# olsonanl/signature_kmers

Hardware: AMD Instinct MI355X
Metric: k-mers/sec (extract+hash+count) at 1/2/4/8 GPUs; achieved HBM GB/s % (higher is better)
Workload: dtype u8

## Files before the change

signature_kmers_amd/__init__.py:

```python
from __future__ import annotations

import ctypes as C
import os
from dataclasses import dataclass

import numpy as np

__all__ = [
    "SkmError", "lib", "K", "UNDEFINED_FUNCTION", "STORED_DTYPE", "CALL_DTYPE",
    "SignatureBuilder", "KeptKmers", "CmphKmerDb", "FunctionCaller", "mph_build",
    "kmer_to_str", "str_to_kmer", "keys_from_strings", "device_count", "MatrixDistance", "SeqIdMap",
    "matrix_tile_rows",
]

K = 8
UNDEFINED_FUNCTION = 0xFFFF
_HERE = os.path.dirname(os.path.abspath(__file__))
LIB_PATH = os.environ.get("SKM_LIB_PATH") or os.path.join(_HERE, "libskm.so")

STORED_DTYPE = np.dtype([("avg_from_end", "<u2"), ("function_index", "<u2"), ("mean", "<u2"),
                         ("median", "<u2"), ("var", "<u2")])
CALL_DTYPE = np.dtype([("start", "<u4"), ("end", "<u4"), ("count", "<i4"), ("function_index", "<u2"),
                       ("pad", "<u2"), ("protein_length_median", "<u4"),
                       ("protein_length_med_avg_dev", "<f4")])
# ... 280 lines not shown
            return {}
        ms = (C.c_float * n)()
        cnt = (C.c_uint64 * n)()
        buf = C.create_string_buffer(64 * n + 64)
        lib().skm_build_kernel_timings(self._h, buf, len(buf), ms, cnt, n)
        names = buf.value.decode().split("\n")[:n]
        return {names[i]: (float(ms[i]), int(cnt[i])) for i in range(n)}

    def set_option(self, name: str, value: int):
        _check(lib().skm_build_set_option(self._h, name.encode(), int(value)))

    def passes(self) -> int:
        return self.counters()["passes"]

    def counters(self) -> dict:
        v = (C.c_uint64 * 48)()
        n = lib().skm_build_counters(self._h, v, 48)
        names = ["windows", "kept", "overflow_subbuckets", "chain_jobs", "chain_samples", "sequences", "grouped",
                 "overflow_elements", "overflow_kept", "big_groups", "big_kept", "passes", "valid", "giant_chains",
                 "giant_max", "redone", "cap_overflow_scratch", "cap_split", "cap_long_samples", "cap_long_jobs",
                 "demand_overflow_scratch", "demand_split", "demand_long_samples", "demand_long_jobs",
                 "long_samples", "routed", "add_batch_us", "prepare_upload_us", "prepare_plan_us", "prepare_rest_us",
                 "pass_groups", "add_pack_us", "add_dma_wait_us", "finish_us", "finish_wait_us", "finish_copy_us",
                 "finish_chunks", "finish_select_dev_us", "finish_sort_dev_us", "finish_gather_dev_us",
                 "finish_d2h_dev_us", "finish_max_chunk", "finish_wide_index", "kept_cap",
                 "free_after_prepare", "recs_rot", "overflow_light_subbuckets", "overflow_light_elements"]
        return {names[i]: int(v[i]) for i in range(n)}

    def debug_jobs(self, k: int = 64) -> list:
        v = (C.c_uint32 * k)()
        _check(lib().skm_build_debug_jobs(self._h, v, k))
        return [int(x) for x in v]

    def debug_overflow(self, k: int = 4096) -> list:
        v = (C.c_uint32 * k)()
        n = lib().skm_build_debug_overflow(self._h, v, k)
        return [int(x) for x in v[:min(max(n, 0), k)]]

    def debug_stamps(self, enable: bool) -> list:
        v = (C.c_uint64 * 32)()
        _check(lib().skm_build_debug_stamps(self._h, 1 if enable else 0, v, 32))
# ... 554 lines not shown
```

signature_kmers_amd/csrc/skm_build.hip:

```cpp
#include <hip/hip_runtime.h>

#include <algorithm>
#include <type_traits>
#include <chrono>
#include <cmath>
#include <cstdio>
#include <cstdlib>
#include <cstring>
#include <deque>
#include <functional>
#include <memory>
#include <numeric>
#include <string>
#include <thread>
#include <vector>

#include "skm_common.h"
#include "skm_pool.h"
#include "skm_output.h"
#include "skm_util.h"

#if defined(SKM_WITH_RCCL)
#include <rccl/rccl.h>
#endif
// ... 342 lines not shown
            }
}

__device__ __forceinline__ void stats_small(GRes& r, uint32_t x0, uint32_t x1, uint32_t n) {
    r.median = 0;
    r.var = 0;
    if (n == 2) {
        const uint16_t sum = (uint16_t)(x0 + x1);
        const double mean = (double)sum / 2.0;
        const double tmp = (double)x1 - mean;
        const double v = 0.0 * 1.0 / 2.0 + tmp * tmp / 1.0;
        r.var = d2u16(v);
    }
}

__device__ __forceinline__ void mark_seq(uint8_t* f, uint32_t s) {
    const uintptr_t p = reinterpret_cast<uintptr_t>(f);
    if (p & 1u) {
        uint32_t* w = reinterpret_cast<uint32_t*>(p & ~(uintptr_t)1) + (s >> 5);
        const uint32_t m = 1u << (s & 31u);
        if (!(*w & m)) atomicOr(w, m);
    } else {
        f[s] = 1;
    }
}

template <int N>
__device__ __forceinline__ void mark_seqs(uint8_t* f, int flag_check, const uint32_t (&s)[N]) {
    const uintptr_t p = reinterpret_cast<uintptr_t>(f);
    if (p & 1u) {
        uint32_t* w = reinterpret_cast<uint32_t*>(p & ~(uintptr_t)1);
        uint32_t cur[N];
#pragma unroll
        for (int u = 0; u < N; ++u) cur[u] = s[u] != 0xFFFFFFFFu ? w[s[u] >> 5] : 0xFFFFFFFFu;
#pragma unroll
        for (int u = 0; u < N; ++u) {
            const uint32_t m = 1u << (s[u] & 31u);
            if (!(cur[u] & m)) atomicOr(w + (s[u] >> 5), m);
        }
    } else {
        uint8_t cur[N];
#pragma unroll
        for (int u = 0; u < N; ++u) cur[u] = s[u] != 0xFFFFFFFFu && flag_check ? f[s[u]] : (uint8_t)(s[u] == 0xFFFFFFFFu);
#pragma unroll
        for (int u = 0; u < N; ++u)
            if (cur[u] == 0) f[s[u]] = 1;
    }
}

template <int N, class V>
__device__ GRes group_thread(const V& v, uint64_t a, uint32_t c, const uint32_t* __restrict__ glen,
                             uint8_t* __restrict__ flags) {
    GRes r;
    r.kept = false;
    uint32_t fn[N], of[N];
#pragma unroll
    for (int t = 0; t < N; ++t) {
        if ((uint32_t)t < c) {
            fn[t] = v.func(a + t);
            of[t] = (uint32_t)(v.lov(a + t) & 0xFFFFu);
        } else {
            fn[t] = 0x10000u;
            of[t] = 0x10000u;
        }
    }
    uint32_t best_f = fn[0], best_c = 0, rb = 0, run_s = 0;
#pragma unroll
// ... 34 lines not shown
            sum += len;
            const uint32_t q = rb + best_c - 1 - t;
            if (q == 0) lr0 = len;
            if (q == 1) lr1 = len;
        }
    }
    r.mean = d2u16((double)(uint16_t)sum / (double)best_c);
    r.median = 0;
    r.var = 0;
    if (best_c <= 2) stats_small(r, lr0, lr1, best_c);
    return r;
}

template <class V>
__device__ GRes group_wave(const V& v, uint64_t a, uint32_t c, const uint32_t* __restrict__ glen,
                           uint8_t* __restrict__ flags) {
    const uint32_t lane = threadIdx.x & 63u;
    GRes r;
    r.kept = false;
    uint32_t best_f = 0, best_c = 0, rb = 0, run_s = 0;
    uint32_t run_f = v.func(a);
    for (uint32_t base = 0; base < c; base += 64) {
        const uint32_t t = base + lane;
        const bool valid = t < c;
        const uint32_t f = valid ? v.func(a + t) : 0xFFFFFFFFu;
        const uint32_t fp = (valid && t > 0) ? v.func(a + t - 1) : 0xFFFFFFFFu;
        uint64_t m = __ballot(valid && t > 0 && f != fp);
        while (m) {
            const int q = __ffsll((long long)m) - 1;
            m &= m - 1;
            const uint32_t pos = base + (uint32_t)q;
// ... 76 lines not shown
}

__device__ __forceinline__ uint32_t wg_min(uint32_t x, uint32_t* s_wave) {
    const uint32_t lane = threadIdx.x & 63u, wave = threadIdx.x >> 6, nw = blockDim.x >> 6;
    x = wave_min(x);
    if (lane == 0) s_wave[wave] = x;
    __syncthreads();
    uint32_t t = 0xFFFFFFFFu;
    for (uint32_t w = 0; w < nw; ++w) t = min(t, s_wave[w]);
    __syncthreads();
    return t;
}

template <class V>
__device__ bool group_block(const V& v, uint64_t a, uint32_t c, const uint32_t* __restrict__ glen,
                            uint8_t* __restrict__ flags, uint32_t* heads, uint32_t hcap, uint32_t* s_wave, GRes& r) {
    const uint32_t tid = threadIdx.x, nt = blockDim.x;
    r.kept = false;
    uint32_t H = 0;
    for (uint32_t t0 = 0; t0 < c; t0 += nt) {
        const uint32_t t = t0 + tid;
        const bool head = t < c && (t == 0 || v.func(a + t) != v.func(a + t - 1));
        uint32_t tot;
        const uint32_t pos = wg_exclusive_scan(head ? 1u : 0u, s_wave, tot);
        if (head && H + pos < hcap) heads[H + pos] = t;
        H += tot;
    }
    if (H > hcap) return false;
    __syncthreads();
    uint32_t lmax = 0;
    for (uint32_t j = tid; j < H; j += nt) lmax = max(lmax, (j + 1 < H ? heads[j + 1] : c) - heads[j]);
// ... 48 lines not shown
    RUN_LONG_WANT = 12,
    RUN_LONG_WANTJ = 13,
    RUN_ACC_LIGHT_SUB = 14,
    RUN_ACC_LIGHT_ELEMS = 15,
    RUN_ACC_NOVF = 16,
    RUN_ACC_JOBS = 17,
    RUN_ACC_LENS = 18,
    RUN_ACC_OVF_ELEMS = 19,
    RUN_ACC_OVF_KEPT = 20,
    RUN_ACC_BIG = 21,
    RUN_ACC_BIG_KEPT = 22,
    RUN_ACC_GROUPED = 23,
    RUN_LAST_NOVF = 24,
    RUN_LAST_JOBS = 25,
    RUN_NLOC = 26,
    RUN_SLOTS = 64
};
constexpr unsigned long long RUN_F_ARENA = 1;
constexpr unsigned long long RUN_F_RERUN = 2;
constexpr unsigned long long RUN_F_CAP = 4;
enum : uint32_t {
    PLAN_NOVF = 0,
    PLAN_NSPLIT = 1,
    PLAN_NHEAVY = 2,
    PLAN_SKIP = 3,
    PLAN_Q_SPLIT = 4,
    PLAN_Q_HEAVY = 5,
    PLAN_Q_REST = 6,
    PLAN_Q_LIGHT = 7,
    PLAN_SLOTS = 8
// ... 1536 lines not shown
    uint64_t* recs_hi;
    const uint64_t* recs_lo;
    uint64_t* tmp_hi;
    uint64_t* tmp_lo;
    const uint64_t* bstart;
    const uint64_t* seg_start;
    const uint32_t* seg_len;
    uint32_t nsrc;
    uint32_t* sub_tab;
    unsigned long long* kept_ctr;

    uint32_t nbuckets;
    uint32_t bucket_base;
    int rem_bits;
    const uint32_t* glen;
    uint8_t* flags;
    unsigned long long* ctr;
    uint64_t* out_keys;
    skm_stored_kmer_data* out_data;
    Job* jobs;
    uint32_t* lens;
    OvfEntry* ovf;
    uint32_t ovf_cap;
    unsigned long long* stamps;
    uint64_t* big_desc;
    uint32_t big_cap;
    unsigned long long* big_ctr;
    int prio;
    int pshift;
    int flag_check;
    const uint32_t* skip;
// ... 134 lines not shown
        const uint32_t g = L.big[q];
        rep = L.glist[g];
        a = L.goff[rep];
        c = (g + 1 < G ? L.goff[L.glist[g + 1]] : M) - a;
    }
    const bool real = gv && m < c;
    uint64_t key = ~0ull;
    uint32_t pay = 0;
    if (real) {
        const uint32_t j = L.order[a + m];
        const uint64_t hj = L.hi[j], lj = L.lo[j];
        key = ((hj & 0xFFFFull) << 48) | (lj >> 16);
        pay = (uint32_t)(hj >> 47);
    }
    key = seg_bitonic64<S>(key, pay, m);
    const uint32_t f = (uint32_t)(key >> 48);
    const uint32_t fprev = (uint32_t)__shfl_up((int)f, 1, 64);
    const bool head = !real || m == 0 || f != fprev;
    const uint64_t H = __ballot(head);
    const uint64_t above = lane == 63 ? 0ull : (H & ~((2ull << lane) - 1ull));
    const uint32_t nh = above ? (uint32_t)__ffsll((long long)above) - 1u : 64u;
    const uint32_t rlen = min(nh, sbase + c) - lane;
    const uint32_t v = (real && head) ? ((rlen << 16) | (0xFFFFu - f)) : 0u;
    const uint32_t best = seg_reduce_max<S>(v);
    const uint32_t cbest = best >> 16, bf = 0xFFFFu - (best & 0xFFFFu);
    const bool kept = gv && !((float)cbest < float(c) * 0.8f);
    const bool inrun = real && f == bf;
    const uint32_t len16 = pay >> 1;
    const uint32_t sum = seg_reduce_sum<S>(inrun ? len16 : 0u);
    const uint32_t i = (uint32_t)(key & ((1u << ELEM_I_BITS) - 1));
    const uint32_t off = real ? ((len16 - i) & 0xFFFFu) : 0x10000u;
    const uint32_t osort = seg_bitonic32<S>(off, m);
    const uint32_t avg = (uint32_t)__shfl((int)osort, (int)(sbase + (c >> 1)), 64);
    const uint64_t R = __ballot(inrun);
    const uint64_t segmask = (S == 64) ? ~0ull : (((1ull << S) - 1ull) << sbase);
    const uint64_t Rs = R & segmask;
    const uint32_t rs = Rs ? (uint32_t)__ffsll((long long)Rs) - 1u : sbase;
    const uint32_t s = (uint32_t)(key >> ELEM_I_BITS) & ((1u << ELEM_S_BITS) - 1u);
    const uint32_t fl = (A.flag_check && real && A.flags) ? A.flags[s] : 0u;
    const uint32_t len = (pay & 1u) ? A.glen[s] : len16;
    if (kept && real && fl == 0 && A.flags) mark_seq(A.flags, s);
    const uint32_t x0 = (uint32_t)__shfl((int)len, (int)(rs + cbest - 1), 64);
    const uint32_t x1 = (uint32_t)__shfl((int)len, (int)rs, 64);
    if (kept && inrun && cbest >= 3) L.lens32[2 * a + (rs + cbest - 1 - lane)] = len;
    if (kept && m == 0) {
        GRes r;
        r.kept = true;
        r.best_f = bf;
        r.cbest = cbest;
        r.avg = avg;
        r.mean = d2u16((double)(uint16_t)sum / (double)cbest);
        stats_small(r, x0, cbest == 2 ? x1 : 0u, cbest);
        const uint64_t h43 = key_h43(hprefix, (L.hi[rep] >> 16) & REM_MASK, A.rem_bits, A.pshift);
        L.hi[rep] = kept_hi(h43, r.avg);
        if (cbest >= 3) {
            jobinfo[rep] = (a << 16) | JOB_KEPT | cbest;
            fmean[rep] = bf | ((uint32_t)r.mean << 16);
        } else {
            jobinfo[rep] = JOB_KEPT;
// ... 287 lines not shown
    return L;
}

__global__ __launch_bounds__(BPK_THREADS, BPK_WAVES_EU) void k_bucket_process(BucketArgs A) {
    static_assert(CAP % BPK_THREADS == 0, "emit assigns CAP / BPK_THREADS elements per thread");
    __shared__ SubMem s_mem;
    __shared__ uint32_t s_sub[(1 << MAX_B2) + 1];
    if (A.skip && *A.skip) return;
    SubLds L = sub_lds(s_mem);

    const uint32_t bucket = blockIdx.x;
    if (bucket >= A.nbuckets) return;
    const uint64_t r0 = A.bstart[bucket], r1 = A.bstart[bucket + 1];
    const uint64_t n = r1 - r0;
    if (n == 0) return;
    const uint64_t hprefix = (uint64_t)(A.bucket_base + bucket) << A.rem_bits;
    if (A.prio == 1) __builtin_amdgcn_s_setprio(1);
    if (A.prio == 2) __builtin_amdgcn_s_setprio(2);
    if (A.prio >= 3) __builtin_amdgcn_s_setprio(3);

    const bool direct = n <= (uint64_t)CAP && A.nsrc == 1;
    uint32_t nsub = 1;
    if (!direct) {
        const uint32_t* tab = A.sub_tab + (uint64_t)bucket * SUB_TAB;
        nsub = tab[0];
        for (uint32_t d = threadIdx.x; d <= nsub; d += blockDim.x) s_sub[d] = tab[1 + d];
        __syncthreads();
        SKM_STAMP(9);
    }
    struct Batch {
// ... 36 lines not shown
    uint64_t lens_off;
    uint32_t n;
    uint16_t avg, func, mean, pad0;
    uint32_t pad1;
};
static_assert(sizeof(BigOut) == 32, "BigOut layout");

struct BigArgs {
    const uint64_t* desc;
    const unsigned long long* ndesc;
    uint32_t cap;
    const uint64_t* recs_hi;
    const uint64_t* tmp_hi;
    const uint64_t* recs_lo;
    const uint64_t* tmp_lo;
    uint8_t* flags;
    BigOut* out;
};

template <int E>
__device__ __forceinline__ uint32_t ballot_count(const bool (&p)[E]) {
    uint32_t n = 0;
#pragma unroll
    for (int e = 0; e < E; ++e) n += (uint32_t)__popcll(__ballot(p[e]));
    return n;
}

template <int E, int D>
__device__ __forceinline__ void bitonic_cross(uint64_t (&ky)[E], bool take_min) {
#pragma unroll
    for (int e = 0; e < E; ++e) {
// ... 124 lines not shown
        if (t < nb) lens[nb - 1 - t] = (uint32_t)mlen[ky[e] & 0xFFFFu];
    }
    o.n = nb;
    o.avg = (uint16_t)pre;
    o.func = (uint16_t)cand;
    o.mean = d2u16((double)(uint16_t)sum / (double)nb);
    if (lane == 0) B.out[g] = o;
}

constexpr int BIG_WG = 256;

template <bool LARGE>
__global__ __launch_bounds__(BIG_WG, LARGE ? 3 : 4) void k_big_groups(BigArgs B) {
    const uint64_t nd = min((uint64_t)*B.ndesc, (uint64_t)B.cap);
    const uint64_t nw = (uint64_t)gridDim.x * (BIG_WG / 64);
    for (uint64_t g = (uint64_t)blockIdx.x * (BIG_WG / 64) + (threadIdx.x >> 6); g < nd; g += nw) {
        const uint64_t d0 = B.desc[2 * g], d1 = B.desc[2 * g + 1];
        const uint32_t c = (uint32_t)(d0 >> KEY_BITS);
        if (LARGE != (c > 1024u)) continue;
        const uint64_t h43 = d0 & KEY_MASK;
        const uint64_t sel = d1 >> LENS_SEL_SHIFT, off = d1 & LENS_OFF_MASK;
        uint64_t* mem = const_cast<uint64_t*>(sel == LENS_IN_RECS ? B.recs_hi : B.tmp_hi) + off / 2;
        const uint64_t* mlen = (sel == LENS_IN_RECS ? B.recs_lo : B.tmp_lo) + off / 2;
        if constexpr (LARGE) {
            big_group<32>(B, g, mem, mlen, c, h43, d1);
        } else {
            if (c <= 128u) big_group<2>(B, g, mem, mlen, c, h43, d1);
            else if (c <= 256u) big_group<4>(B, g, mem, mlen, c, h43, d1);
            else if (c <= 512u) big_group<8>(B, g, mem, mlen, c, h43, d1);
            else big_group<16>(B, g, mem, mlen, c, h43, d1);
// ... 241 lines not shown

constexpr uint32_t OVF_INLINE_CAP = 32;
constexpr uint32_t OVF_BLOCK_GROUP = 1024;

__global__ __launch_bounds__(BP_THREADS) void k_overflow(BucketArgs A, OvfScratch S, uint32_t* plan, int lo_slot,
                                                          int hi_slot, int q_slot, uint32_t inline_min, int prio) {
    __shared__ uint64_t s_hi[CAP];
    __shared__ uint64_t s_lo[CAP];
    __shared__ __align__(16) uint32_t s_wave[48];
    __shared__ uint32_t s_nbig;
    __shared__ uint32_t s_big[BP_THREADS];
    __shared__ uint32_t s_ninl;
    __shared__ uint64_t s_inl[OVF_INLINE_CAP][2];
    __shared__ uint32_t s_q;
    const uint32_t q_lo = lo_slot < 0 ? 0u : plan[lo_slot], q_hi = plan[hi_slot];
    auto entry = [&](const OvfEntry e) {
        if (e.n == 0) return;
        if ((A.diag & 32) && e.n <= (uint32_t)CAP) return;
        if ((A.diag & 64) && e.n > (uint32_t)CAP) return;
        const uint64_t* src_hi = (e.src ? A.tmp_hi : A.recs_hi) + e.off;
        const uint64_t* src_lo = (e.src ? A.tmp_lo : A.recs_lo) + e.off;
        uint64_t* ghi = S.hi + e.scratch;
        uint64_t* glo = S.lo + e.scratch;
        uint32_t* heads = S.heads + e.scratch;
        uint64_t* jobinfo = S.jobinfo + e.scratch;
        uint32_t* fmean = S.fmean + e.scratch;
        const uint32_t n = e.n;
        uint32_t N = CAP;
        while (N < n) N <<= 1;
        const uint32_t tid = threadIdx.x, nt = blockDim.x;
// ... 427 lines not shown
        __syncthreads();
        const uint32_t q = s_q;
        if (q >= q_hi) break;
        entry(q);
        __syncthreads();
    }
}

__global__ __launch_bounds__(BPK_THREADS, BPK_WAVES_EU) void k_ovf_light(BucketArgs A, uint32_t* plan,
                                                                         unsigned long long* stat) {
    __shared__ SubMem s_mem;
    __shared__ uint32_t s_q;
    if (A.skip && *A.skip) return;
    SubLds L = sub_lds(s_mem);
    const uint32_t q_hi = plan[PLAN_NOVF];
    unsigned long long kept = 0, nel = 0;
    uint32_t nsub = 0;
    for (;;) {
        if (threadIdx.x == 0) s_q = atomicAdd(&plan[PLAN_Q_LIGHT], 1u);
        __syncthreads();
        const uint32_t q = s_q;
        if (q >= q_hi) break;
        const OvfEntry e = A.ovf[q];
        if (e.n != 0 && e.n <= (uint32_t)CAP && e.src == 1) {
            const uint64_t hprefix = (uint64_t)(A.bucket_base + e.bucket) << A.rem_bits;
            L.lens_sel = (LENS_IN_TMP << LENS_SEL_SHIFT) | (2 * e.off);
            L.lens32 = reinterpret_cast<uint32_t*>(A.tmp_hi + e.off);
            kept += process_sub(A.tmp_hi + e.off, A.tmp_lo + e.off, e.n, A, hprefix, L);
            if (threadIdx.x == 0) A.ovf[q].n = 0;
            ++nsub;
// ... 120 lines not shown
#pragma unroll
                for (int e = 0; e < E; ++e) {
                    const uint32_t i = (uint32_t)e * 64u + lane;
                    const uint64_t o = xs64(v[e], j);
                    const bool keep_max = ((i & (uint32_t)j) == 0) == ((i & (uint32_t)k) == 0);
                    v[e] = keep_max ? (v[e] > o ? v[e] : o) : (v[e] < o ? v[e] : o);
                }
            }
        }
    }
}

template <int E>
__device__ __forceinline__ void heavy_bucket_out(const uint32_t* __restrict__ ks, const uint32_t* __restrict__ ls,
                                                 uint32_t a, uint32_t c, uint32_t nb, uint32_t* __restrict__ out,
                                                 uint8_t* flags) {
    const uint32_t lane = threadIdx.x & 63u;
    uint64_t v[E];
#pragma unroll
    for (int e = 0; e < E; ++e) {
        const uint32_t i = (uint32_t)e * 64u + lane;
        v[e] = i < c ? ((uint64_t)ks[a + i] << 32) | ls[a + i] : 0ull;
    }
    wave_sort_desc<E>(v);
#pragma unroll
    for (int e = 0; e < E; ++e) {
        const uint32_t i = (uint32_t)e * 64u + lane;
        if (i < nb) {
            out[i] = (uint32_t)v[e];
            if (flags) mark_seq(flags, (uint32_t)(v[e] >> 32) - 1u);
        }
// ... 2 lines not shown

__global__ __launch_bounds__(HEAVY_WG) void k_heavy(BucketArgs A, HeavyArgs H) {
    static_assert(RBINS <= HEAVY_WG, "one radix bin per thread in the scan");
    __shared__ uint32_t s_hist[RBINS], s_run[RBINS + 48];
    __shared__ uint32_t s_wc[HEAVY_WG / 64][RBINS];
    __shared__ __align__(16) uint32_t s_wave[48];
    __shared__ uint32_t s_bm[2 * (HEAVY_WG / 64)];
    __shared__ uint32_t s_cur, s_sel[3], s_key;
    __shared__ uint32_t s_fb[HV_FT];
    __shared__ uint32_t s_bk[HV_NBK];
    __shared__ uint32_t s_oh[256], s_ol[256];
    static_assert(HV_FT == HV_NBK, "s_fb doubles as the per-bucket best counts");
    const uint32_t tid = threadIdx.x, nt = blockDim.x, lane = tid & 63u, wave = tid >> 6, nw = nt >> 6;
    const uint64_t lt = (1ull << lane) - 1ull;
    const uint32_t nkeys = (uint32_t)*H.nkeys;
    uint32_t tag = 0;
    for (uint32_t q = tid; q < (HEAVY_WG / 64) * RBINS; q += nt) (&s_wc[0][0])[q] = 0;
    __syncthreads();
    constexpr uint32_t U = SPLIT_U;
    for (;;) {
        __syncthreads();
        if (tid == 0) s_key = (uint32_t)min((unsigned long long)nkeys, atomicAdd(H.queue, 1ull));
        __syncthreads();
        const uint32_t q = s_key;
        if (q >= nkeys) break;
        const HeavyKey K = H.keys[q];
        const uint64_t* rec = H.rec + K.off;
        const uint32_t* rlen = H.len + K.off;
        const uint32_t n = K.n;
        uint32_t best_f = 0, cb = 0, NBK = 0;
// ... 500 lines not shown
    for (uint32_t s = blockIdx.x * blockDim.x + threadIdx.x; s < nseq; s += gridDim.x * blockDim.x) {
        uint32_t f = meta[s].func;
        if (f < nf) {
            if (lds)
                atomicAdd(&s_h[f], 1u);
            else
                atomicAdd(&swf[f], 1u);
        }
    }
    __syncthreads();
    if (lds)
        for (uint32_t f = threadIdx.x; f < nf; f += blockDim.x)
            if (s_h[f]) atomicAdd(&swf[f], s_h[f]);
}

__global__ void k_flags_from_bits(const uint32_t* __restrict__ bits, uint32_t nseq, uint8_t* __restrict__ flags) {
    for (uint32_t w = blockIdx.x * blockDim.x + threadIdx.x; w < (nseq + 31) / 32; w += gridDim.x * blockDim.x) {
        const uint32_t v = bits[w];
        const uint32_t n = min(32u, nseq - 32 * w);
        uint8_t* o = flags + 32 * (uint64_t)w;
        for (uint32_t t = 0; t < n; ++t) o[t] = (uint8_t)((v >> t) & 1u);
    }
}

__global__ void k_count_flags(const uint8_t* __restrict__ flags, uint32_t nseq, unsigned long long* __restrict__ out) {
    uint32_t local = 0;
    for (uint32_t s = blockIdx.x * blockDim.x + threadIdx.x; s < nseq; s += gridDim.x * blockDim.x) local += flags[s] ? 1u : 0u;
#pragma unroll
    for (int d = 32; d > 0; d >>= 1) local += __shfl_down(local, d, 64);
    if ((threadIdx.x & 63) == 0 && local) atomicAdd(out, (unsigned long long)local);
}
// ... 115 lines not shown
    int overlap = 0;
    int chain_cus = 0;
    int side_cus = 0;
    int serial_overflow = 0;
    int flag_check = 0;
    int partition_round = 0;
    int stage_round = 1;
    int lane_long = 1 << 20;
    int lane_grid = 256;
    int chain_queue = 0;
    int lane_streams = 1;
    int lane_tail = 1 << 16;
    int sub_target = 0;
    int heavy_lsd = 0;
    int flag_bits = 1;
    int diag = 0;
    int handoff_index_limit = 0;
    int handoff_max_chunk = 0;
};

}

using namespace skm;

struct ChainSet {
    DevBuf hist, offs, sorted, long_off;
};

struct skm_build {
    skm_build_opts opts{};
    int device = 0;
    hipStream_t stream = nullptr;
    struct EvSet {
        hipEvent_t ev[13] = {}, o[3] = {}, o3[3] = {};
    };
    std::deque<EvSet> evsets;
    hipEvent_t* ev = nullptr;
    hipEvent_t* ev_o = nullptr;
    hipEvent_t* ev_o3 = nullptr;
    float last_ms[15] = {};
    uint64_t ovf_elems = 0, ovf_kept = 0, ovf_light_sub = 0, ovf_light_elems = 0;

    uint8_t* st_pin[2] = {};
    size_t st_fill[2] = {};
    hipEvent_t st_ev[2] = {};
    bool st_busy[2] = {};
    int st_cur = 0;
    uint64_t rp_total = 0;
    uint64_t rp_dev = 0;
    uint64_t res_cap = 0;
    std::vector<SeqMeta> h_meta;
    std::vector<uint32_t> h_seqid;
    std::unique_ptr<HostPool> pool;
    HandoffStats handoff;
    std::vector<uint32_t> h_keep;
    std::vector<uint64_t> h_cum;
// ... 907 lines not shown
                b->rot = true;
            } else {
                size_t fr = 0, tot = 0;
                SKM_HIP(hipMemGetInfo(&fr, &tot));
                const uint64_t held = (uint64_t)b->d_keys.bytes + (uint64_t)b->d_data.bytes;
                const uint64_t need = 16 * W + 32 * W + (1ull << 30) + 18 * (b->valid_total / 4);
                if ((uint64_t)fr + held > need) {
                    b->d_recs_hi2.ensure(8 * W);
                    b->d_recs_lo2.ensure(8 * W);
                    b->rot = true;
                }
            }
        }
        size_arena(b);
        b->d_flags.ensure(std::max<uint64_t>(b->n_total, 1));
        b->d_flagbits.ensure(4 * ((b->n_total + 31) / 32 + 1));
        b->overlap = false;
        if (b->tune.overlap && b->world == 1 && b->pass_bits > 0) {
            size_t fr = 0, tot = 0;
            SKM_HIP(hipMemGetInfo(&fr, &tot));
            const uint64_t need = 16 * std::max<uint64_t>(b->pass_max, 1) + 16 * b->cap_local;
            if (b->d_recs_hi2.bytes >= 8 * std::max<uint64_t>(b->pass_max, 1) && b->d_tmp_hi2.bytes >= 8 * b->cap_local) {
                b->overlap = true;
            } else if ((uint64_t)fr > need + tot / 10) {
                b->d_recs_hi2.ensure(8 * std::max<uint64_t>(b->pass_max, 1));
                b->d_recs_lo2.ensure(8 * std::max<uint64_t>(b->pass_max, 1));
                b->d_tmp_hi2.ensure(8 * b->cap_local);
                b->d_tmp_lo2.ensure(8 * b->cap_local);
                b->overlap = true;
            }
            if (b->overlap) b->d_ovf2b.ensure(sizeof(OvfEntry) * std::max<uint64_t>(b->ovf_cap, 1));
// ... 355 lines not shown
    A.recs_hi = multi ? b->d_rhi.as<uint64_t>() : recs_hi(b, pass);
    A.recs_lo = multi ? b->d_rlo.as<uint64_t>() : recs_lo(b, pass);
    A.tmp_hi = tmp_hi(b, pass);
    A.tmp_lo = tmp_lo(b, pass);
    A.bstart = multi ? b->d_vstart.as<uint64_t>() : b->d_bstart.as<uint64_t>();
    A.seg_start = multi ? b->d_seg_start.as<uint64_t>() : nullptr;
    A.seg_len = multi ? b->d_seg_len.as<uint32_t>() : nullptr;
    A.nsrc = multi ? (uint32_t)b->world : 1u;
    A.sub_tab = b->d_sub_tab.as<uint32_t>();
    A.kept_ctr = b->d_ctr.as<unsigned long long>();
    A.nbuckets = NB1;
    A.bucket_base = (pass << (b->owner_bits + b->b1_bits)) | ((uint32_t)b->rank << b->b1_bits);
    A.rem_bits = KEY_BITS - b->pass_bits - b->owner_bits - b->b1_bits;
    A.pshift = KEY_BITS - b->pass_bits;
    A.glen = b->d_glen.as<uint32_t>();
    A.flags = (b->tune.diag & 1) ? nullptr
              : b->tune.flag_bits ? reinterpret_cast<uint8_t*>(reinterpret_cast<uintptr_t>(b->d_flagbits.p) | 1u)
                                  : b->d_flags.as<uint8_t>();
    A.flag_check = b->tune.flag_bits ? 0 : b->tune.flag_check;
    A.ctr = ctr_d;
    A.out_keys = b->d_keys.as<uint64_t>();
    A.out_data = b->d_data.as<skm_stored_kmer_data>();
    A.jobs = b->d_jobs.as<Job>();
    A.lens = b->d_lens.as<uint32_t>();
    A.ovf = b->d_ovf.as<OvfEntry>();
    A.ovf_cap = (uint32_t)b->ovf_cap;
    A.prio = b->tune.bucket_prio;
    A.stamps = nullptr;
    A.big_desc = b->d_big_desc.as<uint64_t>();
    A.big_cap = (uint32_t)std::min<uint64_t>(b->big_cap, 0xFFFFFFFFull);
    A.big_ctr = ctr_d + 5;
    A.skip = nullptr;
    A.sub_target = (uint32_t)std::max(0, b->tune.sub_target);
// ... 289 lines not shown
}

void begin_run(skm_build* b) {
    hipStream_t st = b->stream;
    alloc_caps(b);
    b->chainq_next = 0;
    b->emit_q = -1;
    b->giant_timed = false;
    b->tail_pending = false;
    b->tail_issue = nullptr;
    SKM_HIP(hipEventRecord(b->ev_start, st));
    SKM_HIP(hipMemsetAsync(b->d_ctr.p, 0, 3 * 256, st));
    b->ovf_pending[0] = b->ovf_pending[1] = false;
    SKM_HIP(hipMemsetAsync(b->d_run.p, 0, 8 * RUN_SLOTS, st));
    SKM_HIP(hipMemsetAsync(b->d_flags.p, 0, b->n_total ? b->n_total : 1, st));
    if (b->tune.flag_bits) SKM_HIP(hipMemsetAsync(b->d_flagbits.p, 0, 4 * ((b->n_total + 31) / 32 + 1), st));
    b->d_gstat.ensure(16);
    SKM_HIP(hipMemsetAsync(b->d_gstat.p, 0, 16, st));
    if (b->tune.poison_jobs && b->pass_bits && b->long_jobs_cap)
        hipLaunchKernelGGL(k_poison_jobs, dim3(256), dim3(256), 0, st, b->d_long_jobs.as<Job>(), b->long_jobs_cap,
                           reinterpret_cast<uint64_t>(b->d_long_arena.p), (uint32_t)b->kept_cap,
                           b->d_data.as<skm_stored_kmer_data>());
    if (b->pass_bits) {
        const uint32_t P = 1u << b->pass_bits;
        SKM_LAUNCH(b, k_pass_ids, dim3(b->sel_wg), dim3(256), 4u * P + (b->route ? (1u << BLOOM_BITS) / 8 : 0u), st,
                   b->d_res.as<uint8_t>(), b->rp, b->pass_bits, 0, b->d_ids.as<uint8_t>(), nullptr,
                   b->route ? b->d_bloom.as<uint32_t>() : nullptr, P, b->d_selrows.as<uint32_t>(), b->sel_span,
                   route_arg(b));
        SKM_LAUNCH(b, k_sel_scan, dim3(P), dim3(1024), 0, st, b->d_selrows.as<uint32_t>(), b->sel_wg, P,
                   b->d_seloff.as<uint64_t>(), b->d_npos.as<unsigned long long>(), b->pass_max,
                   b->d_run.as<unsigned long long>());
// ... 68 lines not shown
                   b->d_long_jobs.as<Job>(), rng, rng + 1, b->long_jobs_cap, b->d_data.as<skm_stored_kmer_data>(),
                   lane_max, q);
        b->lane_used[ls] = true;
    }
    SKM_HIP(hipGetLastError());
}

void phase_stats(skm_build* b) {
    hipStream_t st = b->stream;
    const uint32_t F = b->opts.n_functions;
    SKM_HIP(hipEventRecord(b->ev_tail[0], st));
    join_tail(b);
    drain_overflow(b);
    if (b->tune.flag_bits && b->n_total)
        SKM_LAUNCH(b, k_flags_from_bits, dim3(1024), dim3(256), 0, st, b->d_flagbits.as<uint32_t>(),
                   (uint32_t)b->n_total, b->d_flags.as<uint8_t>());
    SKM_HIP(hipMemsetAsync(b->d_dfunc.p, 0, sizeof(uint32_t) * (F ? F : 1), st));
    SKM_HIP(hipMemsetAsync(b->d_swf.p, 0, sizeof(uint32_t) * (F ? F : 1), st));
    const size_t lds_f = F <= 16384 ? sizeof(uint32_t) * F : 0;
    if (b->pass_bits) flush_long_chains(b, 16);
    SKM_LAUNCH(b, k_kept_finalize, dim3(2048), dim3(256), lds_f, st, b->d_keys.as<uint64_t>(),
                       b->d_data.as<skm_stored_kmer_data>(), b->d_ctr.as<unsigned long long>(), F,
                       b->d_dfunc.as<uint32_t>());
    if (b->nseq)
        SKM_LAUNCH(b, k_func_hist_seqs, dim3(256), dim3(256), lds_f, st, b->d_meta.as<SeqMeta>(), b->nseq, F,
                           b->d_swf.as<uint32_t>());
    if (b->pass_bits) {
        for (int k = 0; k < skm_build::LANE_ST; ++k) {
            if (!b->lane_used[k]) continue;
            SKM_HIP(hipEventRecord(b->lane_ev[k], b->lane_st[k]));
            SKM_HIP(hipStreamWaitEvent(st, b->lane_ev[k], 0));
// ... 52 lines not shown
        SKM_HIP(hipEventElapsedTime(&b->last_ms[14], b->ev_start, b->ev_giant[1]));
    }
    b->long_samples = R[RUN_LONG_CUR];
    kt_collect(b);
    b->n_overflow = (uint32_t)R[RUN_ACC_NOVF];
    b->n_overflow_last = (uint32_t)R[RUN_LAST_NOVF];
    b->n_jobs = R[RUN_ACC_JOBS];
    b->n_jobs_last = R[RUN_LAST_JOBS];
    b->n_lens = R[RUN_ACC_LENS];
    b->ovf_elems = R[RUN_ACC_OVF_ELEMS];
    b->ovf_kept = R[RUN_ACC_OVF_KEPT];
    b->n_big = R[RUN_ACC_BIG];
    b->big_kept = R[RUN_ACC_BIG_KEPT];
    b->ovf_light_sub = R[RUN_ACC_LIGHT_SUB];
    b->ovf_light_elems = R[RUN_ACC_LIGHT_ELEMS];
    b->n_local = R[RUN_ACC_GROUPED];
    b->ran = true;
}

void grow_caps(skm_build* b) {
    auto grow = [](uint64_t& cap, uint64_t dem) {
        if (dem > cap) cap = dem + dem / 8 + 1024;
    };
    grow(b->tot_cap, b->demand[0]);
    grow(b->split_cap, b->demand[1]);
    grow(b->long_cap, b->demand[2]);
    grow(b->long_jobs_cap, b->demand[3]);
    SKM_HIP(hipDeviceSynchronize());
    alloc_caps(b);
}
// ... 452 lines not shown
               : n == "giant_passes" ? &t.giant_passes
               : n == "heavy_lsd" ? &t.heavy_lsd
               : n == "prefetch" ? &t.prefetch
               : n == "overflow_grid" ? &t.ovf_grid
               : n == "split_grid" ? &t.split_grid
               : n == "chain_grid" ? &t.chain_grid
               : n == "chain_batches" ? &t.chain_batches
               : n == "chain_streams" ? &t.chain_streams
               : n == "poison_jobs" ? &t.poison_jobs
               : n == "route_heavy_min" ? &t.route_heavy_min
               : n == "stage_round" ? &t.stage_round
               : n == "partition_round" ? &t.partition_round
               : n == "flag_check" ? &t.flag_check
               : n == "diag" ? &t.diag
               : n == "flag_bits" ? &t.flag_bits
               : n == "sub_target" ? &t.sub_target
               : n == "lane_long" ? &t.lane_long
               : n == "lane_grid" ? &t.lane_grid
               : n == "lane_tail" ? &t.lane_tail
               : n == "lane_streams" ? &t.lane_streams
               : n == "chain_queue" ? &t.chain_queue
               : n == "serial_overflow" ? &t.serial_overflow
               : n == "overlap" ? &t.overlap
               : n == "heavy_grid" ? &t.heavy_grid
               : n == "route_vacate" ? &t.route_vacate
               : n == "route_first" ? &t.route_first
               : n == "tail_async" ? &t.tail_async
               : n == "big_grid" ? &t.big_grid
               : n == "big_grid_large" ? &t.big_grid_large
               : n == "big_split" ? &t.big_split
// ... 123 lines not shown
    SKM_API_BEGIN
    SKM_CHECK(mismatches && nm, SKM_E_ARG, "bad argument");
    DevBuf d;
    d.ensure(8);
    SKM_HIP(hipMemset(d.p, 0, 8));
    hipLaunchKernelGGL(k_div_check, dim3((uint32_t)ceil_div(nm, 256)), dim3(256), 0, 0, nm, per,
                       d.as<unsigned long long>());
    SKM_HIP(hipGetLastError());
    SKM_HIP(hipMemcpy(mismatches, d.p, 8, hipMemcpyDeviceToHost));
    SKM_API_END
}

int skm_build_counters(skm_build* b, uint64_t* out, int cap) {
    if (!b || !out) return SKM_E_ARG;
    auto us = [](double sec) { return (uint64_t)(sec * 1e6); };
    const uint64_t v[48] = {b->n_windows, b->n_kept, b->n_overflow, b->n_jobs, b->n_lens, b->nseq, b->n_local,
                            b->ovf_elems, b->ovf_kept, b->n_big, b->big_kept, 1ull << b->pass_bits, b->valid_total,
                            b->giant_jobs, b->giant_max, b->n_redo, b->tot_cap, b->split_cap, b->long_cap,
                            b->long_jobs_cap, b->demand[0], b->demand[1], b->demand[2], b->demand[3],
                            b->long_samples, b->routed, us(b->add_s), us(b->prep_upload_s), us(b->prep_plan_s),
                            us(b->prep_rest_s), b->pass_bits ? (1ull << b->pass_bits) / b->emit_g : 0ull, us(b->add_pack_s),
                            us(b->add_wait_s), us(b->handoff.total_s), us(b->handoff.wait_s),
                            us(b->handoff.copy_s), b->handoff.chunks, (uint64_t)(1e3 * b->handoff.select_ms),
                            (uint64_t)(1e3 * b->handoff.sort_ms), (uint64_t)(1e3 * b->handoff.gather_ms),
                            (uint64_t)(1e3 * b->handoff.d2h_ms), b->handoff.max_chunk,
                            (uint64_t)b->handoff.wide_index, b->kept_cap, b->free_after_prepare,
                            (uint64_t)b->rot, b->ovf_light_sub, b->ovf_light_elems};
    int n = std::min(cap, 48);
    for (int i = 0; i < n; ++i) out[i] = v[i];
    return n;
}

int skm_build_set_kernel_timing(skm_build* b, int enable, const char* only) {
    SKM_API_BEGIN
    SKM_CHECK(b, SKM_E_ARG, "null build");
    b->kt_mode = enable ? 1 : 0;
    b->kt_only = only ? std::string(only) : std::string();
    SKM_API_END
}

int skm_build_kernel_timings(skm_build* b, char* names, size_t names_cap, float* ms, uint64_t* launches, int cap) {
    if (!b) return SKM_E_ARG;
    const int n = (int)b->kt_names.size();
// ... 302 lines not shown
```

Measured before the change: 11.75 billion.

## Add hierarchical summary bitmap and early-out for sequence flag marking

Adds a second-level summary bitmap over the per-sequence flag bit words, plus a header holding a count of full words. Marking checks the summary first and skips the word read and atomicOr when a 32-sequence word is already full. Each kernel also drops flag marking entirely once every word is full. This targets redundant global loads and atomics on hot flag words, at the cost of extra atomics when a word fills, a larger flag buffer, and an init kernel.

```diff
diff --git a/signature_kmers_amd/__init__.py b/signature_kmers_amd/__init__.py
--- a/signature_kmers_amd/__init__.py
+++ b/signature_kmers_amd/__init__.py
@@ -318,8 +318,8 @@
         return self.counters()["passes"]
 
     def counters(self) -> dict:
-        v = (C.c_uint64 * 48)()
-        n = lib().skm_build_counters(self._h, v, 48)
+        v = (C.c_uint64 * 49)()
+        n = lib().skm_build_counters(self._h, v, 49)
         names = ["windows", "kept", "overflow_subbuckets", "chain_jobs", "chain_samples", "sequences", "grouped",
                  "overflow_elements", "overflow_kept", "big_groups", "big_kept", "passes", "valid", "giant_chains",
                  "giant_max", "redone", "cap_overflow_scratch", "cap_split", "cap_long_samples", "cap_long_jobs",
@@ -328,7 +328,8 @@
                  "pass_groups", "add_pack_us", "add_dma_wait_us", "finish_us", "finish_wait_us", "finish_copy_us",
                  "finish_chunks", "finish_select_dev_us", "finish_sort_dev_us", "finish_gather_dev_us",
                  "finish_d2h_dev_us", "finish_max_chunk", "finish_wide_index", "kept_cap",
-                 "free_after_prepare", "recs_rot", "overflow_light_subbuckets", "overflow_light_elements"]
+                 "free_after_prepare", "recs_rot", "overflow_light_subbuckets", "overflow_light_elements",
+                 "flag_full_words"]
         return {names[i]: int(v[i]) for i in range(n)}
 
     def debug_jobs(self, k: int = 64) -> list:
diff --git a/signature_kmers_amd/csrc/skm_build.hip b/signature_kmers_amd/csrc/skm_build.hip
--- a/signature_kmers_amd/csrc/skm_build.hip
+++ b/signature_kmers_amd/csrc/skm_build.hip
@@ -380,43 +380,91 @@
     }
 }
 
-__device__ __forceinline__ void mark_seq(uint8_t* f, uint32_t s) {
-    const uintptr_t p = reinterpret_cast<uintptr_t>(f);
+constexpr uint32_t FLAG_HDR_WORDS = 32;
+constexpr uint32_t FLAG_HDR_FULL = 0;
+constexpr uint32_t FLAG_HDR_NWORDS = 1;
+#ifndef SKM_FLAG_EARLYOUT
+#define SKM_FLAG_EARLYOUT 1
+#endif
+struct FlagRef {
+    uint8_t* p;
+    uint32_t* sum;
+    __host__ __device__ explicit operator bool() const { return p != nullptr; }
+};
+
+__device__ __forceinline__ FlagRef flags_live(FlagRef f) {
+#if SKM_FLAG_EARLYOUT
+    if (f.p && f.sum) {
+        const uint32_t* h = f.sum - FLAG_HDR_WORDS;
+        if (__builtin_nontemporal_load(h + FLAG_HDR_FULL) == h[FLAG_HDR_NWORDS]) f.p = nullptr;
+    }
+#endif
+    return f;
+}
+
+__device__ __forceinline__ bool flag_sum_set(const uint32_t* sum, uint32_t s) {
+    return (sum[s >> 10] >> ((s >> 5) & 31u)) & 1u;
+}
+
+__device__ __forceinline__ void mark_bit(uint32_t* w, uint32_t* sum, uint32_t s, uint32_t cur) {
+    const uint32_t m = 1u << (s & 31u);
+    if (!(cur & m)) {
+        const uint32_t old = atomicOr(w + (s >> 5), m);
+        if (sum && old != 0xFFFFFFFFu && (old | m) == 0xFFFFFFFFu) {
+            atomicOr(sum + (s >> 10), 1u << ((s >> 5) & 31u));
+            atomicAdd(sum - FLAG_HDR_WORDS + FLAG_HDR_FULL, 1u);
+        }
+    } else if (sum && cur == 0xFFFFFFFFu) {
+        atomicOr(sum + (s >> 10), 1u << ((s >> 5) & 31u));
+    }
+}
+
+__device__ __forceinline__ void mark_seq(FlagRef f, uint32_t s) {
+    const uintptr_t p = reinterpret_cast<uintptr_t>(f.p);
     if (p & 1u) {
-        uint32_t* w = reinterpret_cast<uint32_t*>(p & ~(uintptr_t)1) + (s >> 5);
-        const uint32_t m = 1u << (s & 31u);
-        if (!(*w & m)) atomicOr(w, m);
+        if (f.sum && flag_sum_set(f.sum, s)) return;
+        uint32_t* w = reinterpret_cast<uint32_t*>(p & ~(uintptr_t)1);
+        mark_bit(w, f.sum, s, w[s >> 5]);
     } else {
-        f[s] = 1;
+        f.p[s] = 1;
     }
 }
 
 template <int N>
-__device__ __forceinline__ void mark_seqs(uint8_t* f, int flag_check, const uint32_t (&s)[N]) {
-    const uintptr_t p = reinterpret_cast<uintptr_t>(f);
+__device__ __forceinline__ void mark_seqs(FlagRef f, int flag_check, const uint32_t (&s)[N]) {
+    const uintptr_t p = reinterpret_cast<uintptr_t>(f.p);
     if (p & 1u) {
         uint32_t* w = reinterpret_cast<uint32_t*>(p & ~(uintptr_t)1);
-        uint32_t cur[N];
-#pragma unroll
-        for (int u = 0; u < N; ++u) cur[u] = s[u] != 0xFFFFFFFFu ? w[s[u] >> 5] : 0xFFFFFFFFu;
-#pragma unroll
-        for (int u = 0; u < N; ++u) {
-            const uint32_t m = 1u << (s[u] & 31u);
-            if (!(cur[u] & m)) atomicOr(w + (s[u] >> 5), m);
-        }
+        uint32_t t[N], cur[N];
+#pragma unroll
+        for (int u = 0; u < N; ++u) t[u] = s[u];
+        if (f.sum) {
+            bool any = false;
+#pragma unroll
+            for (int u = 0; u < N; ++u)
+                if (t[u] != 0xFFFFFFFFu && flag_sum_set(f.sum, t[u])) t[u] = 0xFFFFFFFFu;
+#pragma unroll
+            for (int u = 0; u < N; ++u) any |= t[u] != 0xFFFFFFFFu;
+            if (!any) return;
+        }
+#pragma unroll
+        for (int u = 0; u < N; ++u) cur[u] = t[u] != 0xFFFFFFFFu ? w[t[u] >> 5] : 0xFFFFFFFFu;
+#pragma unroll
+        for (int u = 0; u < N; ++u)
+            if (t[u] != 0xFFFFFFFFu) mark_bit(w, f.sum, t[u], cur[u]);
     } else {
         uint8_t cur[N];
 #pragma unroll
-        for (int u = 0; u < N; ++u) cur[u] = s[u] != 0xFFFFFFFFu && flag_check ? f[s[u]] : (uint8_t)(s[u] == 0xFFFFFFFFu);
+        for (int u = 0; u < N; ++u) cur[u] = s[u] != 0xFFFFFFFFu && flag_check ? f.p[s[u]] : (uint8_t)(s[u] == 0xFFFFFFFFu);
 #pragma unroll
         for (int u = 0; u < N; ++u)
-            if (cur[u] == 0) f[s[u]] = 1;
+            if (cur[u] == 0) f.p[s[u]] = 1;
     }
 }
 
 template <int N, class V>
 __device__ GRes group_thread(const V& v, uint64_t a, uint32_t c, const uint32_t* __restrict__ glen,
-                             uint8_t* __restrict__ flags) {
+                             FlagRef flags) {
     GRes r;
     r.kept = false;
     uint32_t fn[N], of[N];
@@ -481,7 +529,7 @@
 
 template <class V>
 __device__ GRes group_wave(const V& v, uint64_t a, uint32_t c, const uint32_t* __restrict__ glen,
-                           uint8_t* __restrict__ flags) {
+                           FlagRef flags) {
     const uint32_t lane = threadIdx.x & 63u;
     GRes r;
     r.kept = false;
@@ -588,7 +636,7 @@
 
 template <class V>
 __device__ bool group_block(const V& v, uint64_t a, uint32_t c, const uint32_t* __restrict__ glen,
-                            uint8_t* __restrict__ flags, uint32_t* heads, uint32_t hcap, uint32_t* s_wave, GRes& r) {
+                            FlagRef flags, uint32_t* heads, uint32_t hcap, uint32_t* s_wave, GRes& r) {
     const uint32_t tid = threadIdx.x, nt = blockDim.x;
     r.kept = false;
     uint32_t H = 0;
@@ -667,6 +715,7 @@
     RUN_LAST_NOVF = 24,
     RUN_LAST_JOBS = 25,
     RUN_NLOC = 26,
+    RUN_FLAG_FULL = 27,
     RUN_SLOTS = 64
 };
 constexpr unsigned long long RUN_F_ARENA = 1;
@@ -2233,7 +2282,7 @@
     uint32_t bucket_base;
     int rem_bits;
     const uint32_t* glen;
-    uint8_t* flags;
+    FlagRef flags;
     unsigned long long* ctr;
     uint64_t* out_keys;
     skm_stored_kmer_data* out_data;
@@ -2398,6 +2447,9 @@
         pay = (uint32_t)(hj >> 47);
     }
     key = seg_bitonic64<S>(key, pay, m);
+    const uint32_t s = (uint32_t)(key >> ELEM_I_BITS) & ((1u << ELEM_S_BITS) - 1u);
+    uint32_t fsum = 0u;
+    if (real && A.flags && A.flags.sum) fsum = A.flags.sum[s >> 10] & (1u << ((s >> 5) & 31u));
     const uint32_t f = (uint32_t)(key >> 48);
     const uint32_t fprev = (uint32_t)__shfl_up((int)f, 1, 64);
     const bool head = !real || m == 0 || f != fprev;
@@ -2420,13 +2472,17 @@
     const uint64_t segmask = (S == 64) ? ~0ull : (((1ull << S) - 1ull) << sbase);
     const uint64_t Rs = R & segmask;
     const uint32_t rs = Rs ? (uint32_t)__ffsll((long long)Rs) - 1u : sbase;
-    const uint32_t s = (uint32_t)(key >> ELEM_I_BITS) & ((1u << ELEM_S_BITS) - 1u);
-    const uint32_t fl = (A.flag_check && real && A.flags) ? A.flags[s] : 0u;
+    const uint32_t fl = (A.flag_check && real && A.flags) ? A.flags.p[s] : 0u;
     const uint32_t len = (pay & 1u) ? A.glen[s] : len16;
-    if (kept && real && fl == 0 && A.flags) mark_seq(A.flags, s);
+    const bool mk = kept && real && fl == 0 && A.flags;
+    if (mk && !A.flags.sum) mark_seq(A.flags, s);
     const uint32_t x0 = (uint32_t)__shfl((int)len, (int)(rs + cbest - 1), 64);
     const uint32_t x1 = (uint32_t)__shfl((int)len, (int)rs, 64);
     if (kept && inrun && cbest >= 3) L.lens32[2 * a + (rs + cbest - 1 - lane)] = len;
+    if (mk && A.flags.sum && !fsum) {
+        uint32_t* w = reinterpret_cast<uint32_t*>(reinterpret_cast<uintptr_t>(A.flags.p) & ~(uintptr_t)1);
+        mark_bit(w, A.flags.sum, s, w[s >> 5]);
+    }
     if (kept && m == 0) {
         GRes r;
         r.kept = true;
@@ -2744,6 +2800,7 @@
     const uint64_t r0 = A.bstart[bucket], r1 = A.bstart[bucket + 1];
     const uint64_t n = r1 - r0;
     if (n == 0) return;
+    A.flags = flags_live(A.flags);
     const uint64_t hprefix = (uint64_t)(A.bucket_base + bucket) << A.rem_bits;
     if (A.prio == 1) __builtin_amdgcn_s_setprio(1);
     if (A.prio == 2) __builtin_amdgcn_s_setprio(2);
@@ -2810,7 +2867,7 @@
     const uint64_t* tmp_hi;
     const uint64_t* recs_lo;
     const uint64_t* tmp_lo;
-    uint8_t* flags;
+    FlagRef flags;
     BigOut* out;
 };
 
@@ -2965,6 +3022,7 @@
 __global__ __launch_bounds__(BIG_WG, LARGE ? 3 : 4) void k_big_groups(BigArgs B) {
     const uint64_t nd = min((uint64_t)*B.ndesc, (uint64_t)B.cap);
     const uint64_t nw = (uint64_t)gridDim.x * (BIG_WG / 64);
+    B.flags = flags_live(B.flags);
     for (uint64_t g = (uint64_t)blockIdx.x * (BIG_WG / 64) + (threadIdx.x >> 6); g < nd; g += nw) {
         const uint64_t d0 = B.desc[2 * g], d1 = B.desc[2 * g + 1];
         const uint32_t c = (uint32_t)(d0 >> KEY_BITS);
@@ -3236,6 +3294,7 @@
     __shared__ uint64_t s_inl[OVF_INLINE_CAP][2];
     __shared__ uint32_t s_q;
     const uint32_t q_lo = lo_slot < 0 ? 0u : plan[lo_slot], q_hi = plan[hi_slot];
+    A.flags = flags_live(A.flags);
     auto entry = [&](const OvfEntry e) {
         if (e.n == 0) return;
         if ((A.diag & 32) && e.n <= (uint32_t)CAP) return;
@@ -3693,6 +3752,7 @@
     if (A.skip && *A.skip) return;
     SubLds L = sub_lds(s_mem);
     const uint32_t q_hi = plan[PLAN_NOVF];
+    A.flags = flags_live(A.flags);
     unsigned long long kept = 0, nel = 0;
     uint32_t nsub = 0;
     for (;;) {
@@ -3843,7 +3903,7 @@
 template <int E>
 __device__ __forceinline__ void heavy_bucket_out(const uint32_t* __restrict__ ks, const uint32_t* __restrict__ ls,
                                                  uint32_t a, uint32_t c, uint32_t nb, uint32_t* __restrict__ out,
-                                                 uint8_t* flags) {
+                                                 FlagRef flags) {
     const uint32_t lane = threadIdx.x & 63u;
     uint64_t v[E];
 #pragma unroll
@@ -3876,6 +3936,7 @@
     const uint32_t tid = threadIdx.x, nt = blockDim.x, lane = tid & 63u, wave = tid >> 6, nw = nt >> 6;
     const uint64_t lt = (1ull << lane) - 1ull;
     const uint32_t nkeys = (uint32_t)*H.nkeys;
+    A.flags = flags_live(A.flags);
     uint32_t tag = 0;
     for (uint32_t q = tid; q < (HEAVY_WG / 64) * RBINS; q += nt) (&s_wc[0][0])[q] = 0;
     __syncthreads();
@@ -4406,7 +4467,19 @@
             if (s_h[f]) atomicAdd(&swf[f], s_h[f]);
 }
 
-__global__ void k_flags_from_bits(const uint32_t* __restrict__ bits, uint32_t nseq, uint8_t* __restrict__ flags) {
+inline uint64_t flag_nwords(uint64_t nseq) { return (nseq + 31) / 32; }
+inline uint64_t flag_sum_word(uint64_t nseq) { return (flag_nwords(nseq) + 1 + 31) / 32 * 32 + FLAG_HDR_WORDS; }
+inline uint64_t flag_bytes(uint64_t nseq) { return 4 * (flag_sum_word(nseq) + flag_nwords(flag_nwords(nseq)) + 1); }
+
+__global__ void k_flagbits_init(uint32_t* __restrict__ bits, uint32_t nseq, uint32_t* __restrict__ sum) {
+    if (blockIdx.x || threadIdx.x) return;
+    if (nseq & 31u) bits[nseq >> 5] = 0xFFFFFFFFu << (nseq & 31u);
+    sum[(int)FLAG_HDR_NWORDS - (int)FLAG_HDR_WORDS] = (nseq + 31) / 32;
+}
+
+__global__ void k_flags_from_bits(const uint32_t* __restrict__ bits, uint32_t nseq, uint8_t* __restrict__ flags,
+                                  const uint32_t* __restrict__ full, unsigned long long* __restrict__ run) {
+    if (full && blockIdx.x == 0 && threadIdx.x == 0) run[RUN_FLAG_FULL] = *full;
     for (uint32_t w = blockIdx.x * blockDim.x + threadIdx.x; w < (nseq + 31) / 32; w += gridDim.x * blockDim.x) {
         const uint32_t v = bits[w];
         const uint32_t n = min(32u, nseq - 32 * w);
@@ -4552,6 +4625,7 @@
     int sub_target = 0;
     int heavy_lsd = 0;
     int flag_bits = 1;
+    int flag_summary = 1;
     int diag = 0;
     int handoff_index_limit = 0;
     int handoff_max_chunk = 0;
@@ -4577,7 +4651,7 @@
     hipEvent_t* ev_o = nullptr;
     hipEvent_t* ev_o3 = nullptr;
     float last_ms[15] = {};
-    uint64_t ovf_elems = 0, ovf_kept = 0, ovf_light_sub = 0, ovf_light_elems = 0;
+    uint64_t ovf_elems = 0, ovf_kept = 0, ovf_light_sub = 0, ovf_light_elems = 0, flag_full_words = 0;
 
     uint8_t* st_pin[2] = {};
     size_t st_fill[2] = {};
@@ -5515,7 +5589,7 @@
         }
         size_arena(b);
         b->d_flags.ensure(std::max<uint64_t>(b->n_total, 1));
-        b->d_flagbits.ensure(4 * ((b->n_total + 31) / 32 + 1));
+        b->d_flagbits.ensure(flag_bytes(b->n_total));
         b->overlap = false;
         if (b->tune.overlap && b->world == 1 && b->pass_bits > 0) {
             size_t fr = 0, tot = 0;
@@ -5901,9 +5975,11 @@
     A.rem_bits = KEY_BITS - b->pass_bits - b->owner_bits - b->b1_bits;
     A.pshift = KEY_BITS - b->pass_bits;
     A.glen = b->d_glen.as<uint32_t>();
-    A.flags = (b->tune.diag & 1) ? nullptr
-              : b->tune.flag_bits ? reinterpret_cast<uint8_t*>(reinterpret_cast<uintptr_t>(b->d_flagbits.p) | 1u)
-                                  : b->d_flags.as<uint8_t>();
+    A.flags.p = (b->tune.diag & 1) ? nullptr
+                : b->tune.flag_bits ? reinterpret_cast<uint8_t*>(reinterpret_cast<uintptr_t>(b->d_flagbits.p) | 1u)
+                                    : b->d_flags.as<uint8_t>();
+    A.flags.sum = b->tune.flag_bits && b->tune.flag_summary ? b->d_flagbits.as<uint32_t>() + flag_sum_word(b->n_total)
+                                                            : nullptr;
     A.flag_check = b->tune.flag_bits ? 0 : b->tune.flag_check;
     A.ctr = ctr_d;
     A.out_keys = b->d_keys.as<uint64_t>();
@@ -6223,7 +6299,12 @@
     b->ovf_pending[0] = b->ovf_pending[1] = false;
     SKM_HIP(hipMemsetAsync(b->d_run.p, 0, 8 * RUN_SLOTS, st));
     SKM_HIP(hipMemsetAsync(b->d_flags.p, 0, b->n_total ? b->n_total : 1, st));
-    if (b->tune.flag_bits) SKM_HIP(hipMemsetAsync(b->d_flagbits.p, 0, 4 * ((b->n_total + 31) / 32 + 1), st));
+    if (b->tune.flag_bits) {
+        SKM_HIP(hipMemsetAsync(b->d_flagbits.p, 0, flag_bytes(b->n_total), st));
+        if (b->tune.flag_summary)
+            SKM_LAUNCH(b, k_flagbits_init, dim3(1), dim3(64), 0, st, b->d_flagbits.as<uint32_t>(), (uint32_t)b->n_total,
+                       b->d_flagbits.as<uint32_t>() + flag_sum_word(b->n_total));
+    }
     b->d_gstat.ensure(16);
     SKM_HIP(hipMemsetAsync(b->d_gstat.p, 0, 16, st));
     if (b->tune.poison_jobs && b->pass_bits && b->long_jobs_cap)
@@ -6322,7 +6403,10 @@
     drain_overflow(b);
     if (b->tune.flag_bits && b->n_total)
         SKM_LAUNCH(b, k_flags_from_bits, dim3(1024), dim3(256), 0, st, b->d_flagbits.as<uint32_t>(),
-                   (uint32_t)b->n_total, b->d_flags.as<uint8_t>());
+                   (uint32_t)b->n_total, b->d_flags.as<uint8_t>(),
+                   b->tune.flag_summary ? b->d_flagbits.as<uint32_t>() + flag_sum_word(b->n_total) - FLAG_HDR_WORDS + FLAG_HDR_FULL
+                                        : nullptr,
+                   b->d_run.as<unsigned long long>());
     SKM_HIP(hipMemsetAsync(b->d_dfunc.p, 0, sizeof(uint32_t) * (F ? F : 1), st));
     SKM_HIP(hipMemsetAsync(b->d_swf.p, 0, sizeof(uint32_t) * (F ? F : 1), st));
     const size_t lds_f = F <= 16384 ? sizeof(uint32_t) * F : 0;
@@ -6405,6 +6489,7 @@
     b->big_kept = R[RUN_ACC_BIG_KEPT];
     b->ovf_light_sub = R[RUN_ACC_LIGHT_SUB];
     b->ovf_light_elems = R[RUN_ACC_LIGHT_ELEMS];
+    b->flag_full_words = R[RUN_FLAG_FULL];
     b->n_local = R[RUN_ACC_GROUPED];
     b->ran = true;
 }
@@ -6887,6 +6972,7 @@
                : n == "flag_check" ? &t.flag_check
                : n == "diag" ? &t.diag
                : n == "flag_bits" ? &t.flag_bits
+               : n == "flag_summary" ? &t.flag_summary
                : n == "sub_target" ? &t.sub_target
                : n == "lane_long" ? &t.lane_long
                : n == "lane_grid" ? &t.lane_grid
@@ -7040,7 +7126,7 @@
 int skm_build_counters(skm_build* b, uint64_t* out, int cap) {
     if (!b || !out) return SKM_E_ARG;
     auto us = [](double sec) { return (uint64_t)(sec * 1e6); };
-    const uint64_t v[48] = {b->n_windows, b->n_kept, b->n_overflow, b->n_jobs, b->n_lens, b->nseq, b->n_local,
+    const uint64_t v[49] = {b->n_windows, b->n_kept, b->n_overflow, b->n_jobs, b->n_lens, b->nseq, b->n_local,
                             b->ovf_elems, b->ovf_kept, b->n_big, b->big_kept, 1ull << b->pass_bits, b->valid_total,
                             b->giant_jobs, b->giant_max, b->n_redo, b->tot_cap, b->split_cap, b->long_cap,
                             b->long_jobs_cap, b->demand[0], b->demand[1], b->demand[2], b->demand[3],
@@ -7051,8 +7137,8 @@
                             (uint64_t)(1e3 * b->handoff.sort_ms), (uint64_t)(1e3 * b->handoff.gather_ms),
                             (uint64_t)(1e3 * b->handoff.d2h_ms), b->handoff.max_chunk,
                             (uint64_t)b->handoff.wide_index, b->kept_cap, b->free_after_prepare,
-                            (uint64_t)b->rot, b->ovf_light_sub, b->ovf_light_elems};
-    int n = std::min(cap, 48);
+                            (uint64_t)b->rot, b->ovf_light_sub, b->ovf_light_elems, b->flag_full_words};
+    int n = std::min(cap, 49);
     for (int i = 0; i < n; ++i) out[i] = v[i];
     return n;
 }
```

Result: no change. 11.70 billion, median of 2 (-0.4%).
